# mpriessner/MultiModalSpectralTransformer

Hardware: NVIDIA B200
Metric: generated SMILES tokens/sec (higher is better)
Workload: dtype bf16

## Files before the change

multimodalspectraltransformer_b200/csrc/engine.cu:

```cuda
#include "engine.cuh"
#include "kernels_simt.cuh"
#include "kernels_tc.cuh"
#include "kernels_decode.cuh"
#include "kernels_ffn.cuh"
#include "kernels_attn5.cuh"
#include "kernels_compact.cuh"
#include "kernels_beam.cuh"

#include <algorithm>
#include <cstdlib>
#include <cstring>

namespace mmt {
thread_local std::string g_last_error;

static const char* kEmbedKeys[5] = {
    "linear_spec_embedding_1H.point_embedding_layer_1H.fc_H",
    "linear_spec_embedding_13C.point_embedding_layer_13C.fc_C",
    "linear_spec_embedding_HSQC.point_embedding_layer_HSQC.fc_HSQC",
    "linear_spec_embedding_COSY.point_embedding_layer_COSY.fc_COSY",
    "linear_spec_embedding_IR.linear_spec_embedding_IR"};
static const char* kEncNames[6] = {"encoder_1H", "encoder_13C", "encoder_HSQC", "encoder_COSY", "encoder_IR", "encoder_cross"};

static void prof_pre(mmt_engine* e, cudaStream_t s) {
// ... 129 lines not shown
        void* fn = nullptr;
        cudaDriverEntryPointQueryResult qres;
        MMT_CUDA(cudaGetDriverEntryPoint("cuTensorMapEncodeTiled", &fn, cudaEnableDefault, &qres));
        if (!fn || qres != cudaDriverEntryPointSuccess) MMT_FAIL("cuTensorMapEncodeTiled not available from the driver");
        g_encode_tiled = (PFN_tmapEncodeTiled)fn;
    }
    const int max_smem = TC_MAX_STAGES * TC_STAGE_BYTES_WSPLIT + 1024;
    MMT_CUDA(cudaFuncSetAttribute(gemm_bf16_tc<TC_EPI_STORE>, cudaFuncAttributeMaxDynamicSharedMemorySize, max_smem));
    MMT_CUDA(cudaFuncSetAttribute(gemm_bf16_tc<TC_EPI_LN>, cudaFuncAttributeMaxDynamicSharedMemorySize, max_smem));
    MMT_CUDA(cudaFuncSetAttribute(attn_encoder_tc5, cudaFuncAttributeMaxDynamicSharedMemorySize, A5_SMEM_BYTES));
    MMT_CUDA(cudaFuncSetAttribute(ffn_fused_tc<TC_EPI_STORE, 1>, cudaFuncAttributeMaxDynamicSharedMemorySize, ff_smem_bytes<1>()));
    MMT_CUDA(cudaFuncSetAttribute(ffn_fused_tc<TC_EPI_LN, 1>, cudaFuncAttributeMaxDynamicSharedMemorySize, ff_smem_bytes<1>()));
    MMT_CUDA(cudaFuncSetAttribute(ffn_fused_tc<TC_EPI_STORE, 0>, cudaFuncAttributeMaxDynamicSharedMemorySize, ff_smem_bytes<0>()));
    MMT_CUDA(cudaFuncSetAttribute(ffn_fused_tc<TC_EPI_LN, 0>, cudaFuncAttributeMaxDynamicSharedMemorySize, ff_smem_bytes<0>()));
    MMT_CUDA(cudaFuncSetAttribute(ffn_fused_tc<TC_EPI_LN, 0, 1>, cudaFuncAttributeMaxDynamicSharedMemorySize, ff_smem_bytes<0, 1>()));
    e->tc_ready = true;
    return 0;
}

static int make_tmap(CUtensorMap* m, const __nv_bfloat16* ptr, int64_t rows, int64_t cols, int64_t ld, int box_rows = TC_BM) {
    if (((uintptr_t)ptr & 15) || (ld * 2) % 16) MMT_FAIL("tensor map: operand must be 16-byte aligned with a 16-byte multiple row pitch");
    cuuint64_t dims[2] = {(cuuint64_t)cols, (cuuint64_t)rows};
    cuuint64_t strides[1] = {(cuuint64_t)ld * 2};
    cuuint32_t box[2] = {(cuuint32_t)TC_BK, (cuuint32_t)box_rows};
    cuuint32_t estr[2] = {1, 1};
    CUresult r = g_encode_tiled(m, CU_TENSOR_MAP_DATA_TYPE_BFLOAT16, 2, (void*)ptr, dims, strides, box, estr, CU_TENSOR_MAP_INTERLEAVE_NONE,
                                CU_TENSOR_MAP_SWIZZLE_128B, CU_TENSOR_MAP_L2_PROMOTION_L2_256B, CU_TENSOR_MAP_FLOAT_OOB_FILL_NONE);
    if (r != CUDA_SUCCESS) MMT_FAIL("cuTensorMapEncodeTiled failed with CUresult " + std::to_string((int)r));
    return 0;
}
// ... 73 lines not shown
    }
    if (pro) {
        if (epi != TC_EPI_LN || p.splits != 1 || !pro->W || !pro->out || p.res != pro->out)
            MMT_FAIL("fused FFN prologue needs the LayerNorm epilogue, a weight and the residual buffer as its output");
        p.pro = pro->Wlo ? 2 : 1; p.pro_bias = pro->bias; p.pro_gamma = pro->gamma; p.pro_beta = pro->beta; p.pro_out = pro->out;
        MMT_TRY(make_tmap(&p.tmP, pro->W, D, D, D));
        if (pro->Wlo) MMT_TRY(make_tmap(&p.tmPlo, pro->Wlo, D, D, D));
    }
    dim3 grid(p.splits, (p.M + TC_BM - 1) / TC_BM);
    if (const char* v = getenv("MMT_FFN_KNOCK")) p.knock = atoi(v);
    prof_pre(e, s);
    if (p.wsplit) {
        if (epi == TC_EPI_LN) launch_kernel(ffn_fused_tc<TC_EPI_LN, 1>, grid, dim3(FF_THREADS), ff_smem_bytes<1>(), s, pdl, p);
        else launch_kernel(ffn_fused_tc<TC_EPI_STORE, 1>, grid, dim3(FF_THREADS), ff_smem_bytes<1>(), s, pdl, p);
    } else {
        if (epi == TC_EPI_LN && p.splits == 1 && p.F % (2 * FF_CH) == 0 && e->use_ffn_wide)
            launch_kernel(ffn_fused_tc<TC_EPI_LN, 0, 1>, grid, dim3(ff_threads<0, 1>()), ff_smem_bytes<0, 1>(), s, pdl, p);
        else if (epi == TC_EPI_LN) launch_kernel(ffn_fused_tc<TC_EPI_LN, 0>, grid, dim3(FF_THREADS), ff_smem_bytes<0>(), s, pdl, p);
        else launch_kernel(ffn_fused_tc<TC_EPI_STORE, 0>, grid, dim3(FF_THREADS), ff_smem_bytes<0>(), s, pdl, p);
    }
    return check_launch(e, "ffn_fused_tc", s, 4.0 * p.M * D * p.F);
}

struct ModeLayout {
    int present[5];
    int S_m[5];
    int n_x[5];
    int off[5];
    int S_total;
    int float_mask;
    int has_MF, has_MS, has_MW;
// ... 736 lines not shown

static int decode_self_tail_layer(const DecOps& o, const LayerW& w, bool bf16) {
    const DecBuffers& b = o.b;
    if (bf16) {
        if (o.e->use_gemm_chain && o.Nw <= 24576) {
            const TcChain ch{o.e->Wb(w.ca_in_w), o.plo(w.ca_in_w), w.ca_in_b, b.qc, D};
            MMT_TRY(o.tc_ln(b.att16, D, w.out_w, w.out_b, D, w.n1_w, w.n1_b, &ch));
        } else {
            MMT_TRY(o.tc_ln(b.att16, D, w.out_w, w.out_b, D, w.n1_w, w.n1_b));
            MMT_TRY(o.tc(b.x16, D, w.ca_in_w, w.ca_in_b, b.qc, nullptr, D, D, 0, 1));
        }
    } else {
        MMT_TRY(o.gemm(b.att, D, w.out_w, nullptr, b.part, D, D, 0, 1));
        MMT_TRY(o.ln(b.part, 1, w.out_b, w.n1_w, w.n1_b));
        MMT_TRY(o.gemm(b.x, D, w.ca_in_w, w.ca_in_b, b.qc, D, D, 0, 1));
    }
    return 0;
}

static int decode_cross_tail_layer(const DecOps& o, const LayerW& w, int l, bool bf16, float* x2 = nullptr) {
    mmt_engine* e = o.e;
    const DecBuffers& b = o.b;
    const int M = (int)o.Nw, F = e->desc.d_ff;
    cudaStream_t s = o.s;
    auto keep_x2 = [&]() -> int {
        if (x2) MMT_CUDA(cudaMemcpyAsync(x2, b.x, (size_t)M * D * sizeof(float), cudaMemcpyDeviceToDevice, s));
        return 0;
    };
    if (bf16) {
        const bool ffn_pro = e->use_ffn_prologue && M >= 2048;
// ... 317 lines not shown
        while (early && !stop && checked_polls < n_polls) { MMT_TRY(check_poll(checked_polls)); ++checked_polls; }
        if ((r.mode == 0) && a.stop_on_all_pad && n_waves > 1) {
            for (int i = 0; i < nl; ++i)
                MMT_CUDA(cudaMemcpyAsync(e->h_pinned + i * 128, lb[i].ctl + 8, r.T * sizeof(int), cudaMemcpyDeviceToHost, s));
            MMT_CUDA(cudaStreamSynchronize(s));
            for (int i = 0; i < nl; ++i) for (int q = 0; q < r.T; ++q) nonpad_total[q] += e->h_pinned[i * 128 + q];
        }
    }
    if (staged) {
        MMT_CUDA(cudaMemcpyAsync(r.tokens, st_tokens, (size_t)r.T * N_total * sizeof(int64_t), cudaMemcpyDeviceToDevice, s));
        if (r.probs) MMT_CUDA(cudaMemcpyAsync(r.probs, st_probs, (size_t)r.T * N_total * sizeof(float), cudaMemcpyDeviceToDevice, s));
    }
    if ((r.mode == 0) && a.stop_on_all_pad && n_waves > 1)
        for (int q = 0; q < r.T; ++q) if (nonpad_total[q] == 0) { steps_done = q + 1; break; }
    if (h_steps) *h_steps = steps_done;
    if (e->ffn_dbg) {
        MMT_CUDA(cudaStreamSynchronize(s));
        for (int bshow : {0, 64, 127}) {
            const long long* d = e->ffn_dbg + bshow * 16;
            fprintf(stderr, "ffn_fused_tc<LN> CTA %d: setup %lld | first acc1 %lld | first convert %lld | chunks 8..15:", bshow, d[1] - d[0], d[2] - d[1], d[3] - d[2]);
            for (int i = 9; i <= 15; ++i) fprintf(stderr, " %lld", d[i] - d[i - 1]);
            fprintf(stderr, " | start->acc2 %lld | tmem->stage %lld | LN rows %lld | total %lld\n", d[4] - d[0], d[5] - d[4], d[6] - d[5], d[7] - d[0]);
        }
    }
    if (e->da_dbg) {
        MMT_CUDA(cudaStreamSynchronize(s));
        const int blocks = (int)std::min<int64_t>(4096, (std::min<int64_t>(N_total, max_wave_seqs) + DA_R - 1) / DA_R);
        for (int bshow : {0, blocks / 2, blocks - 1}) {
            fprintf(stderr, "decode_attn phases, CTA %d:", bshow);
            const int last = e->da_dbg[bshow * 16 + 14] ? 14 : 10;
            for (int i = 1; i <= last; ++i) fprintf(stderr, " %lld", e->da_dbg[bshow * 16 + i] - e->da_dbg[bshow * 16 + i - 1]);
            fprintf(stderr, "  total %lld\n", e->da_dbg[bshow * 16 + last] - e->da_dbg[bshow * 16]);
        }
        for (int bshow : {1, blocks / 2}) {
            const long long* d = e->da_dbg + (1024 + bshow) * 16;
            fprintf(stderr, "decode_attn warp 5, CTA %d: self [K+scores %lld | V+acc %lld | reduce %lld | sync %lld]  cross [loop %lld | reduce %lld | sync %lld]\n", bshow,
                    d[1] - d[0], d[2] - d[1], d[3] - d[2], d[4] - d[3], d[6] - d[5], d[7] - d[6], d[8] - d[7]);
        }
        for (int bshow : {0, 33}) {
// ... 172 lines not shown
    if (getenv("MMT_DENSE_ENCODER")) e->use_compact = false;
    if (getenv("MMT_NO_TC_ATTENTION")) e->use_tc_attention = false;
    if (getenv("MMT_TC5_ATTENTION")) e->use_tc5_attention = true;
    if (const char* v = getenv("MMT_FFN_SPLITS")) { int k = atoi(v); if (k == 1 || k == 2 || k == 4 || k == 8 || k == 16 || k == 32) e->ffn_splits_override = k; }
    if (getenv("MMT_TC_ATTENTION_FP32")) e->tc_attention_fp32 = true;
    if (const char* v = getenv("MMT_FUSED_DECODE_ROWS")) e->fused_decode_rows = atoi(v);
    if (getenv("MMT_DEC_FFN_TWO_TERM")) e->dec_ffn_single = false;
    if (getenv("MMT_DEC_PROJ_TWO_TERM")) e->dec_proj_single = false;
    if (const char* v = getenv("MMT_PDL_ROWS")) e->pdl_rows = atoi(v);
    if (getenv("MMT_NO_GEMM_CHAIN")) e->use_gemm_chain = false;
    if (getenv("MMT_NO_FFN_WIDE")) e->use_ffn_wide = false;
    if (getenv("MMT_NO_KV_EPILOGUE")) e->use_kv_epilogue = false;
    if (getenv("MMT_KV_HEAD_MAJOR")) e->kv_tok_major = false;
    if (getenv("MMT_CLUSTER_FFN")) e->use_cluster_ffn = true;
    if (getenv("MMT_NO_FFN_PROLOGUE")) e->use_ffn_prologue = false;
    if (getenv("MMT_ENC_FFN_SINGLE")) e->enc_ffn_single = true;
    if (const char* v = getenv("MMT_DECODE_LANES_LARGE")) e->decode_lanes_large = std::max(1, atoi(v));
    if (const char* v = getenv("MMT_MAX_WAVE_SEQS")) e->max_wave_seqs = std::max(1, atoi(v));
    if (n_floats != e->reg.total) { delete e; MMT_FAIL("weight blob has " + std::to_string(n_floats) + " floats, expected " + std::to_string(build_registry(*desc).total)); }
    auto fail = [&](const std::string& m) { mmt_destroy(e); g_last_error = m; return 1; };
    if (cudaMalloc(&e->w32, n_floats * sizeof(float)) != cudaSuccess) return fail("cudaMalloc weights failed");
    if (cudaMalloc(&e->w16, n_floats * sizeof(__nv_bfloat16)) != cudaSuccess) return fail("cudaMalloc bf16 weights failed");
    if (cudaMemcpy(e->w32, h_weights, n_floats * sizeof(float), cudaMemcpyHostToDevice) != cudaSuccess) return fail("weight H2D copy failed");
    if (cudaMalloc(&e->w16lo, n_floats * sizeof(__nv_bfloat16)) != cudaSuccess) return fail("cudaMalloc bf16 weights (low term) failed");
    f32_to_bf16_split<<<(unsigned)((n_floats + 255) / 256), 256>>>(e->w32, n_floats, e->w16, e->w16lo);
    if (cudaDeviceSynchronize() != cudaSuccess) return fail(std::string("bf16 weight conversion failed: ") + cudaGetErrorString(cudaGetLastError()));
    if (cudaMallocHost(&e->h_pinned, 1024 * sizeof(int32_t)) != cudaSuccess) return fail("cudaMallocHost failed");
    for (int k = 0; k < 6; ++k) {
        e->enc[k].resize(desc->n_enc_layers);
        for (int l = 0; l < desc->n_enc_layers; ++l) fill_layer(e, e->enc[k][l], std::string(kEncNames[k]) + ".layers." + std::to_string(l), false);
// ... 431 lines not shown
            return check_launch(e, "f32_to_bf16", s);
        }
        MMT_CUDA(cudaMemcpyAsync(b.att, src, bytes, cudaMemcpyDeviceToDevice, s));
        return 0;
    };
    const DecOps o{e, b, R, false, s};
    const LayerW& w = e->dec[layer];
    MMT_CUDA(cudaMemcpyAsync(b.x, d_x, bytes, cudaMemcpyDeviceToDevice, s));
    MMT_TRY(load_att(d_att_self));
    MMT_TRY(decode_self_tail_layer(o, w, bf16));
    MMT_CUDA(cudaMemcpyAsync(d_x1, b.x, bytes, cudaMemcpyDeviceToDevice, s));
    MMT_CUDA(cudaMemcpyAsync(d_qc, b.qc, bytes, cudaMemcpyDeviceToDevice, s));
    MMT_TRY(load_att(d_att_cross));
    MMT_TRY(decode_cross_tail_layer(o, w, layer, bf16, d_x2));
    MMT_CUDA(cudaMemcpyAsync(d_out, b.x, bytes, cudaMemcpyDeviceToDevice, s));
    return 0;
}

int32_t mmt_encoder_layer(mmt_engine* e, int32_t stack, int32_t layer, const float* d_x, int64_t rows, int32_t B, int32_t S,
                          const float* d_key_bias, const int32_t* d_row_start, const int32_t* d_cnt, const int32_t* d_kidx,
                          const int32_t* d_nk, int32_t kstride, int32_t precision, float* d_qkv, float* d_att, float* d_out,
                          void* stream) {
    if (!e || !d_x || !d_out) MMT_FAIL("null argument");
    const mmt_model_desc& d = e->desc;
    if (stack < 0 || stack > 5) MMT_FAIL("mmt_encoder_layer: stack must be in [0, 5]");
    if (layer < 0 || layer >= d.n_enc_layers) MMT_FAIL("mmt_encoder_layer: layer out of range");
    if (B <= 0 || B > 65535 || S <= 0 || rows <= 0 || rows > 0x7fffffff) MMT_FAIL("mmt_encoder_layer: empty or oversized batch");
    if (precision != MMT_PREC_FP32 && precision != MMT_PREC_BF16) MMT_FAIL("bad precision");
    const bool ragged = d_key_bias == nullptr;
    if (ragged && (!d_row_start || !d_cnt || !d_kidx || !d_nk || kstride <= 0)) MMT_FAIL("mmt_encoder_layer: the ragged layout needs row_start, cnt, kidx, nk and kstride");
// ... 107 lines not shown
```

multimodalspectraltransformer_b200/csrc/engine.cuh:

```cuda
#pragma once
#include <mutex>
#include <string>
#include <unordered_map>
#include <vector>

#include "../../include/mmt_b200.h"
#include "common.cuh"

namespace mmt {

extern thread_local std::string g_last_error;

#define MMT_FAIL(msg)                                                                   \
    do {                                                                                \
        ::mmt::g_last_error = std::string(__FILE__) + ":" + std::to_string(__LINE__) + ": " + (msg); \
        return 1;                                                                       \
    } while (0)
#define MMT_CUDA(call)                                                                  \
    do {                                                                                \
        cudaError_t err__ = (call);                                                     \
        if (err__ != cudaSuccess) MMT_FAIL(std::string(#call) + " -> " + cudaGetErrorString(err__)); \
    } while (0)
#define MMT_TRY(call)                                                                   \
    do {                                                                                \
// ... 84 lines not shown
    __nv_bfloat16* w16lo = nullptr;
    std::vector<mmt::LayerW> enc[6];
    std::vector<mmt::LayerW> dec;
    char* arena = nullptr;
    size_t arena_bytes = 0;
    int64_t launches = 0;
    bool use_graph = true;
    int fused_decode_rows = 2048;
    int max_wave_seqs = 0;
    bool enc_ffn_single = false;
    bool use_ffn_prologue = true;
    bool use_cluster_ffn = false;
    bool kv_tok_major = true;
    bool use_kv_epilogue = true;
    bool use_ffn_wide = true;
    bool use_gemm_chain = true;
    bool dec_proj_single = true;
    bool sample_ready = false;
    bool dec_ffn_single = true;
    bool use_compact = true;
    struct GraphEntry { std::vector<uint64_t> key; cudaGraphExec_t exec; int64_t launches_per_group; uint64_t stamp; };
    std::vector<GraphEntry> graph_cache;
    uint64_t graph_cache_clock = 0;
    bool use_graph_cache = true;
    bool use_tc_attention = true;
    bool use_tc5_attention = false;
    bool tc_attention_fp32 = false;
    int ffn_splits_override = 0;
    bool use_enc_streams = true;
    cudaStream_t enc_stream[5] = {nullptr, nullptr, nullptr, nullptr, nullptr};
    cudaEvent_t enc_ev[6] = {nullptr, nullptr, nullptr, nullptr, nullptr, nullptr};
    int graph_steps = 16;
    int pdl_rows = 4096;
    bool use_pdl = true;
    cudaStream_t cap_stream[4] = {nullptr, nullptr, nullptr, nullptr};
    cudaEvent_t lane_ev[4] = {nullptr, nullptr, nullptr, nullptr};
    int decode_lanes = 2;
    int decode_lanes_large = 1;
    long long* ffn_dbg = nullptr;
    long long* da_dbg = nullptr;
    bool da_ready = false;
    bool tc_ready = false;
    cudaEvent_t poll_ev[2] = {nullptr, nullptr};
    int32_t* h_pinned = nullptr;
    struct ProfRecord { const char* name; cudaEvent_t a, b; double work; };
    bool profiling = false;
    std::pair<cudaEvent_t, cudaEvent_t> prof_open{nullptr, nullptr};
    std::vector<ProfRecord> prof_records;

    std::mutex mu;
    cudaEvent_t last_use = nullptr;
    cudaStream_t last_stream = nullptr;
    bool last_use_valid = false;

// ... 5 lines not shown
```

multimodalspectraltransformer_b200/csrc/kernels_ffn.cuh:

```cuda
#pragma once
#include "kernels_tc.cuh"

namespace mmt {

constexpr int FF_CH = 64;
constexpr int FF_THREADS = TC_THREADS + 32;
template <int WS, int WIDE> constexpr int ff_threads();
constexpr int FF_X_BYTES = 2 * TC_SLAB_BYTES;
constexpr int FF_H_BYTES = TC_SLAB_BYTES;
constexpr int FF_W1_HALF = FF_CH * 128;
constexpr int FF_W1_STAGE = 2 * TC_SLAB_BYTES;
constexpr int FF_W2_STAGE = 2 * TC_SLAB_BYTES;
constexpr int FF_MAX_F = 2048;
template <int WS, int WIDE> struct FfCfg;
template <> struct FfCfg<1, 0> {
    static constexpr int CH = FF_CH, NB = 2, NS = 2;
    static constexpr int EW = TC_EPI_WARPS;
    static constexpr int W1_STAGE = FF_W1_STAGE, W2_STAGE = FF_W2_STAGE;
    static constexpr int W1_SLAB = TC_SLAB_BYTES;
    static constexpr int W2_KSLAB = 2 * TC_SLAB_BYTES;
    static constexpr int H_BYTES = FF_H_BYTES;
    static constexpr int ACC1_STRIDE = 2 * FF_CH, ACC2_COL = 256;
};
template <> struct FfCfg<0, 0> {
// ... 324 lines not shown
        const float* st = stage_q + (hf * RPW) * TC_LDS;
        if (EPI == TC_EPI_LN) epi_rows_ln(p, st, m0 + q * 32 + hf * RPW, RPW, lane, nullptr, 0, &pre);
        else epi_rows_store(p, st, m0 + q * 32 + hf * RPW, RPW, 0, split, lane);
        if (threadIdx.x == 64) FF_STAMP(6);
    }
    tc_fence_before();
    __syncthreads();
    if (threadIdx.x == 64) FF_STAMP(7);
#undef FF_STAMP
    if (warp == 1) {
        tc_fence_after();
        tmem_dealloc(tmem_base, FF_TMEM_COLS);
    }
}

}
```

multimodalspectraltransformer_b200/csrc/kernels_tc.cuh:

```cuda
#pragma once
#include <cuda.h>

#include "common.cuh"

namespace mmt {

constexpr int TC_BM = 128, TC_BN = 128, TC_BK = 64;
constexpr int TC_SLAB_BYTES = TC_BM * TC_BK * 2;
constexpr int TC_STAGE_BYTES = 2 * TC_SLAB_BYTES;
constexpr int TC_STAGE_BYTES_WSPLIT = 3 * TC_SLAB_BYTES;
constexpr int TC_LDS = TC_BN + 4;
constexpr int TC_STAGING_BYTES = TC_BM * TC_LDS * 4;
constexpr int TC_EPI_WARPS = 8;
constexpr int TC_THREADS = 64 + TC_EPI_WARPS * 32;
constexpr int TC_MAX_STAGES = 4;

enum { TC_EPI_STORE = 0, TC_EPI_LN = 1 };

struct TcGemmParams {
    CUtensorMap tmA;
    CUtensorMap tmW;
    CUtensorMap tmW2;
    int wsplit;
    int M, N, K;
// ... 75 lines not shown
__device__ __forceinline__ void umma_commit(uint64_t* bar) {
    asm volatile("tcgen05.commit.cta_group::1.mbarrier::arrive::one.shared::cluster.b64 [%0];" ::"r"(smem_u32(bar)) : "memory");
}
__device__ __forceinline__ void tmem_ld_32x32(uint32_t taddr, uint32_t (&r)[32]) {
    asm volatile(
        "tcgen05.ld.sync.aligned.32x32b.x32.b32 "
        "{%0, %1, %2, %3, %4, %5, %6, %7, %8, %9, %10, %11, %12, %13, %14, %15, "
        "%16, %17, %18, %19, %20, %21, %22, %23, %24, %25, %26, %27, %28, %29, %30, %31}, [%32];"
        : "=r"(r[0]), "=r"(r[1]), "=r"(r[2]), "=r"(r[3]), "=r"(r[4]), "=r"(r[5]), "=r"(r[6]), "=r"(r[7]),
          "=r"(r[8]), "=r"(r[9]), "=r"(r[10]), "=r"(r[11]), "=r"(r[12]), "=r"(r[13]), "=r"(r[14]), "=r"(r[15]),
          "=r"(r[16]), "=r"(r[17]), "=r"(r[18]), "=r"(r[19]), "=r"(r[20]), "=r"(r[21]), "=r"(r[22]), "=r"(r[23]),
          "=r"(r[24]), "=r"(r[25]), "=r"(r[26]), "=r"(r[27]), "=r"(r[28]), "=r"(r[29]), "=r"(r[30]), "=r"(r[31])
        : "r"(taddr) : "memory");
}
__device__ __forceinline__ void tmem_ld_wait() { asm volatile("tcgen05.wait::ld.sync.aligned;" ::: "memory"); }

__device__ __forceinline__ uint64_t umma_desc_sw128(uint32_t smem_addr) {
    uint64_t d = 0;
    d |= (uint64_t)((smem_addr & 0x3FFFFu) >> 4);
    d |= (uint64_t)1 << 16;
    d |= (uint64_t)(1024 >> 4) << 32;
    d |= (uint64_t)1 << 46;
    d |= (uint64_t)2 << 61;
    return d;
}
__host__ __device__ constexpr uint32_t umma_idesc_bf16(int M, int N) {
    return (1u << 4) | (1u << 7) | (1u << 10) | ((uint32_t)(N >> 3) << 17) | ((uint32_t)(M >> 4) << 24);
}

__device__ __forceinline__ uint2 pack_bf16x4(float4 v) {
    __nv_bfloat162 lo = __floats2bfloat162_rn(v.x, v.y), hi = __floats2bfloat162_rn(v.z, v.w);
    return make_uint2(*reinterpret_cast<uint32_t*>(&lo), *reinterpret_cast<uint32_t*>(&hi));
}

constexpr int EPI_ILP = 8;

template <int NCOLS, int NP = 2>
__device__ __forceinline__ void epi_tmem_to_stage(uint32_t tmem_acc, int q, int hf, int lane, float* stage_q) {
#pragma unroll
    for (int cc = 0; cc < NCOLS / 32 / NP; ++cc) {
        const int c = hf * (NCOLS / 32 / NP) + cc;
        uint32_t r[32];
        tmem_ld_32x32(tmem_acc + ((uint32_t)(q * 32) << 16) + (uint32_t)(c * 32), r);
        tmem_ld_wait();
        float* dst = stage_q + lane * TC_LDS + c * 32;
#pragma unroll
        for (int j = 0; j < 8; ++j)
            *reinterpret_cast<float4*>(dst + 4 * j) =
                make_float4(__uint_as_float(r[4 * j]), __uint_as_float(r[4 * j + 1]), __uint_as_float(r[4 * j + 2]), __uint_as_float(r[4 * j + 3]));
    }
}
template <int EW = TC_EPI_WARPS>
__device__ __forceinline__ void epi_bar_sync() { asm volatile("bar.sync 1, %0;" ::"n"(EW * 32) : "memory"); }

__device__ __forceinline__ void warp_sum_ilp(float (&s)[EPI_ILP]) {
#pragma unroll
    for (int o = 16; o > 0; o >>= 1) {
#pragma unroll
        for (int u = 0; u < EPI_ILP; ++u) s[u] += __shfl_xor_sync(0xffffffffu, s[u], o);
    }
}

struct RowStep {
// ... 15 lines not shown

struct LnPre { float4 bias, ga, be; float4 rs[EPI_ILP]; };
template <class P>
__device__ __forceinline__ void epi_ln_prefetch(const P& p, int row0, int nrows, int lane, LnPre& pre) {
    const int col = lane * 4;
    pre.bias = p.bias ? *reinterpret_cast<const float4*>(p.bias + col) : make_float4(0.f, 0.f, 0.f, 0.f);
    pre.ga = *reinterpret_cast<const float4*>(p.gamma + col);
    pre.be = *reinterpret_cast<const float4*>(p.beta + col);
    const int rows = min(nrows, p.M - row0);
    const float* res = p.res + (int64_t)row0 * D + col;
#pragma unroll
    for (int u = 0; u < EPI_ILP; ++u)
        pre.rs[u] = u < rows ? *reinterpret_cast<const float4*>(res + (int64_t)u * D) : make_float4(0.f, 0.f, 0.f, 0.f);
}

template <class P>
__device__ __forceinline__ void epi_rows_ln(const P& p, const float* stage, int row0, int nrows, int lane, uint8_t* a2 = nullptr, int a2_row0 = 0,
                                            const LnPre* pre = nullptr) {
    const int col = lane * 4;
    float4 bias = make_float4(0.f, 0.f, 0.f, 0.f), ga, be;
    if (pre) { bias = pre->bias; ga = pre->ga; be = pre->be; }
    else {
        if (p.bias) bias = *reinterpret_cast<const float4*>(p.bias + col);
        ga = *reinterpret_cast<const float4*>(p.gamma + col);
        be = *reinterpret_cast<const float4*>(p.beta + col);
    }
    const int rows = min(nrows, p.M - row0);
    if (rows <= 0) return;
    const float* res = p.res + (int64_t)row0 * D + col;
    float* const out32 = p.out_f32 ? p.out_f32 + col : nullptr;
    __nv_bfloat16* const out16 = p.out_b16 ? p.out_b16 + col : nullptr;
    const int64_t ld32 = p.ld_f32, ld16 = p.ld_b16;
    const float eps = p.eps;
    RowStep map(p, row0);
    for (int i0 = 0; i0 < rows; i0 += EPI_ILP) {
        float4 v[EPI_ILP];
        float s[EPI_ILP];
#pragma unroll
        for (int u = 0; u < EPI_ILP; ++u) {
            const bool ok = i0 + u < rows;
            const float4 rs = (pre && i0 == 0) ? pre->rs[u]
                            : ok ? *reinterpret_cast<const float4*>(res + (int64_t)(i0 + u) * D) : make_float4(0.f, 0.f, 0.f, 0.f);
            const float4 a = *reinterpret_cast<const float4*>(stage + (i0 + u) * TC_LDS + col);
            v[u] = make_float4(a.x + bias.x + rs.x, a.y + bias.y + rs.y, a.z + bias.z + rs.z, a.w + bias.w + rs.w);
            s[u] = v[u].x + v[u].y + v[u].z + v[u].w;
        }
        warp_sum_ilp(s);
#pragma unroll
        for (int u = 0; u < EPI_ILP; ++u) {
            const float mean = s[u] * (1.0f / D);
            v[u].x -= mean; v[u].y -= mean; v[u].z -= mean; v[u].w -= mean;
            s[u] = v[u].x * v[u].x + v[u].y * v[u].y + v[u].z * v[u].z + v[u].w * v[u].w;
        }
        warp_sum_ilp(s);
#pragma unroll
        for (int u = 0; u < EPI_ILP; ++u) {
            if (i0 + u < rows) {
                const float rstd = rsqrtf(s[u] * (1.0f / D) + eps);
// ... 247 lines not shown
```

Measured before the change: 17.53 million.

## Add persistent fused FFN kernel overlapping prologue GEMM, FFN and LayerNorm across tiles

Adds a persistent ffn_persist_tc kernel that loops over M tiles with one CTA per SM. Within each CTA it runs the prologue out-projection GEMM plus LN, the two FFN GEMMs, and a final LayerNorm done by dedicated row warps directly from TMEM, all double-buffered so tile k+1's prologue overlaps tile k's tail. The aim is to cut per-CTA setup cost (TMEM alloc, barrier init) and keep tensor cores busy across epilogues. It also adds an XOR-swizzled staging layout to avoid shared-memory bank conflicts, a TMEM store helper and debug stamps. The cost is more complex barrier ring logic, and the dedicated LN warps take three passes over TMEM.

New measurement: 16.99 million, median of 6. 0.969x the previous value.

```diff
diff --git a/multimodalspectraltransformer_b200/csrc/engine.cu b/multimodalspectraltransformer_b200/csrc/engine.cu
--- a/multimodalspectraltransformer_b200/csrc/engine.cu
+++ b/multimodalspectraltransformer_b200/csrc/engine.cu
@@ -167,6 +167,7 @@
     MMT_CUDA(cudaFuncSetAttribute(ffn_fused_tc<TC_EPI_STORE, 0>, cudaFuncAttributeMaxDynamicSharedMemorySize, ff_smem_bytes<0>()));
     MMT_CUDA(cudaFuncSetAttribute(ffn_fused_tc<TC_EPI_LN, 0>, cudaFuncAttributeMaxDynamicSharedMemorySize, ff_smem_bytes<0>()));
     MMT_CUDA(cudaFuncSetAttribute(ffn_fused_tc<TC_EPI_LN, 0, 1>, cudaFuncAttributeMaxDynamicSharedMemorySize, ff_smem_bytes<0, 1>()));
+    MMT_CUDA(cudaFuncSetAttribute(ffn_persist_tc, cudaFuncAttributeMaxDynamicSharedMemorySize, ff_smem_bytes<0, 1>()));
     e->tc_ready = true;
     return 0;
 }
@@ -270,7 +271,17 @@
         if (epi == TC_EPI_LN) launch_kernel(ffn_fused_tc<TC_EPI_LN, 1>, grid, dim3(FF_THREADS), ff_smem_bytes<1>(), s, pdl, p);
         else launch_kernel(ffn_fused_tc<TC_EPI_STORE, 1>, grid, dim3(FF_THREADS), ff_smem_bytes<1>(), s, pdl, p);
     } else {
-        if (epi == TC_EPI_LN && p.splits == 1 && p.F % (2 * FF_CH) == 0 && e->use_ffn_wide)
+        const bool wide = epi == TC_EPI_LN && p.splits == 1 && p.F % (2 * FF_CH) == 0 && e->use_ffn_wide;
+        const bool identity_rows = !p.out_rows && p.S_in == p.M && p.stride_s == 1 && p.off == 0;
+        const bool persist = wide && p.pro == 1 && identity_rows && e->use_ffn_persist;
+        if (p.dbg) {
+            e->ffn_dbg_grid = persist ? (int)std::min<int64_t>(grid.y, e->sm_count) : 0;
+            e->ffn_dbg_tiles = (int)grid.y;
+            if (persist && grid.y > 4096) p.dbg = nullptr;
+        }
+        if (persist) {
+            launch_kernel(ffn_persist_tc, dim3((unsigned)std::min<int64_t>(grid.y, e->sm_count)), dim3(fp_threads()), ff_smem_bytes<0, 1>(), s, pdl, p);
+        } else if (wide)
             launch_kernel(ffn_fused_tc<TC_EPI_LN, 0, 1>, grid, dim3(ff_threads<0, 1>()), ff_smem_bytes<0, 1>(), s, pdl, p);
         else if (epi == TC_EPI_LN) launch_kernel(ffn_fused_tc<TC_EPI_LN, 0>, grid, dim3(FF_THREADS), ff_smem_bytes<0>(), s, pdl, p);
         else launch_kernel(ffn_fused_tc<TC_EPI_STORE, 0>, grid, dim3(FF_THREADS), ff_smem_bytes<0>(), s, pdl, p);
@@ -1037,6 +1048,30 @@
         MMT_TRY(o.gemm(b.att, D, w.out_w, nullptr, b.part, D, D, 0, 1));
         MMT_TRY(o.ln(b.part, 1, w.out_b, w.n1_w, w.n1_b));
         MMT_TRY(o.gemm(b.x, D, w.ca_in_w, w.ca_in_b, b.qc, D, D, 0, 1));
+    }
+    return 0;
+}
+
+static int print_ffn_stamps(mmt_engine* e, cudaStream_t s) {
+    MMT_CUDA(cudaStreamSynchronize(s));
+    if (e->ffn_dbg_grid == 0) {
+        for (int bshow : {0, 64, 127}) {
+            const long long* d = e->ffn_dbg + bshow * 16;
+            fprintf(stderr, "ffn_fused_tc<LN> CTA %d: setup %lld | first acc1 %lld | first convert %lld | chunks 8..15:", bshow, d[1] - d[0], d[2] - d[1], d[3] - d[2]);
+            for (int i = 9; i <= 15; ++i) fprintf(stderr, " %lld", d[i] - d[i - 1]);
+            fprintf(stderr, " | start->acc2 %lld | tmem->stage %lld | LN rows %lld | total %lld\n", d[4] - d[0], d[5] - d[4], d[6] - d[5], d[7] - d[0]);
+        }
+        return 0;
+    }
+    const int G = e->ffn_dbg_grid;
+    const long long t0 = e->ffn_dbg[0];
+    for (int t = 0; t < e->ffn_dbg_tiles; t += G) {
+        const long long* d = e->ffn_dbg + (int64_t)t * FP_DBG_SLOTS;
+        fprintf(stderr, "ffn_persist_tc CTA 0 tile %d: prologue GEMM %lld | LN2 %lld..%lld | first acc1 %lld | chunk cadence:", t, d[0] - t0, d[1] - t0, d[2] - t0, d[3] - t0);
+        for (int i = 5; i <= 11; ++i) fprintf(stderr, " %lld", d[i] - d[i - 1]);
+        fprintf(stderr, " | last conversion %lld | LN3 %lld..%lld", d[11] - t0, d[12] - t0, d[13] - t0);
+        if (t + G < e->ffn_dbg_tiles) fprintf(stderr, " | tile period %lld", e->ffn_dbg[(int64_t)(t + G) * FP_DBG_SLOTS + 1] - d[1]);
+        fprintf(stderr, "\n");
     }
     return 0;
 }
@@ -1384,15 +1419,7 @@
     if ((r.mode == 0) && a.stop_on_all_pad && n_waves > 1)
         for (int q = 0; q < r.T; ++q) if (nonpad_total[q] == 0) { steps_done = q + 1; break; }
     if (h_steps) *h_steps = steps_done;
-    if (e->ffn_dbg) {
-        MMT_CUDA(cudaStreamSynchronize(s));
-        for (int bshow : {0, 64, 127}) {
-            const long long* d = e->ffn_dbg + bshow * 16;
-            fprintf(stderr, "ffn_fused_tc<LN> CTA %d: setup %lld | first acc1 %lld | first convert %lld | chunks 8..15:", bshow, d[1] - d[0], d[2] - d[1], d[3] - d[2]);
-            for (int i = 9; i <= 15; ++i) fprintf(stderr, " %lld", d[i] - d[i - 1]);
-            fprintf(stderr, " | start->acc2 %lld | tmem->stage %lld | LN rows %lld | total %lld\n", d[4] - d[0], d[5] - d[4], d[6] - d[5], d[7] - d[0]);
-        }
-    }
+    if (e->ffn_dbg) MMT_TRY(print_ffn_stamps(e, s));
     if (e->da_dbg) {
         MMT_CUDA(cudaStreamSynchronize(s));
         const int blocks = (int)std::min<int64_t>(4096, (std::min<int64_t>(N_total, max_wave_seqs) + DA_R - 1) / DA_R);
@@ -1595,6 +1622,7 @@
     if (getenv("MMT_KV_HEAD_MAJOR")) e->kv_tok_major = false;
     if (getenv("MMT_CLUSTER_FFN")) e->use_cluster_ffn = true;
     if (getenv("MMT_NO_FFN_PROLOGUE")) e->use_ffn_prologue = false;
+    if (getenv("MMT_NO_FFN_PERSIST")) e->use_ffn_persist = false;
     if (getenv("MMT_ENC_FFN_SINGLE")) e->enc_ffn_single = true;
     if (const char* v = getenv("MMT_DECODE_LANES_LARGE")) e->decode_lanes_large = std::max(1, atoi(v));
     if (const char* v = getenv("MMT_MAX_WAVE_SEQS")) e->max_wave_seqs = std::max(1, atoi(v));
@@ -2056,6 +2084,7 @@
     MMT_TRY(load_att(d_att_cross));
     MMT_TRY(decode_cross_tail_layer(o, w, layer, bf16, d_x2));
     MMT_CUDA(cudaMemcpyAsync(d_out, b.x, bytes, cudaMemcpyDeviceToDevice, s));
+    if (e->ffn_dbg && layer == 3) MMT_TRY(print_ffn_stamps(e, s));
     return 0;
 }
 
diff --git a/multimodalspectraltransformer_b200/csrc/engine.cuh b/multimodalspectraltransformer_b200/csrc/engine.cuh
--- a/multimodalspectraltransformer_b200/csrc/engine.cuh
+++ b/multimodalspectraltransformer_b200/csrc/engine.cuh
@@ -122,6 +122,7 @@
     bool kv_tok_major = true;
     bool use_kv_epilogue = true;
     bool use_ffn_wide = true;
+    bool use_ffn_persist = true;
     bool use_gemm_chain = true;
     bool dec_proj_single = true;
     bool sample_ready = false;
@@ -146,6 +147,7 @@
     int decode_lanes = 2;
     int decode_lanes_large = 1;
     long long* ffn_dbg = nullptr;
+    int ffn_dbg_grid = 0, ffn_dbg_tiles = 0;
     long long* da_dbg = nullptr;
     bool da_ready = false;
     bool tc_ready = false;
diff --git a/multimodalspectraltransformer_b200/csrc/kernels_ffn.cuh b/multimodalspectraltransformer_b200/csrc/kernels_ffn.cuh
--- a/multimodalspectraltransformer_b200/csrc/kernels_ffn.cuh
+++ b/multimodalspectraltransformer_b200/csrc/kernels_ffn.cuh
@@ -362,4 +362,331 @@
     }
 }
 
+constexpr int FP_ROW_WARPS = 4;
+constexpr int fp_threads() { return ff_threads<0, 1>() + 32 * FP_ROW_WARPS; }
+constexpr int FP_DBG_SLOTS = 16;
+
+__device__ __forceinline__ void ln_row_thread(const FfnParams& p, uint32_t tacc, int grow) {
+    const bool ok = grow < p.M;
+    const float* res = p.res + (int64_t)(ok ? grow : 0) * D;
+    auto tree = [](float (&s)[16]) {
+#pragma unroll
+        for (int o = 8; o > 0; o >>= 1)
+#pragma unroll
+            for (int L = 0; L < o; ++L) s[L] += s[L + o];
+        return s[0];
+    };
+    float s[16];
+#pragma unroll
+    for (int cg = 0; cg < 4; ++cg) {
+        uint32_t a[32];
+        tmem_ld_32x32(tacc + (uint32_t)(cg * 32), a);
+        tmem_ld_wait();
+#pragma unroll
+        for (int j = 0; j < 8; ++j) {
+            const int col = cg * 32 + 4 * j;
+            const float4 bias = p.bias ? *reinterpret_cast<const float4*>(p.bias + col) : make_float4(0.f, 0.f, 0.f, 0.f);
+            const float4 rs = ok ? *reinterpret_cast<const float4*>(res + col) : make_float4(0.f, 0.f, 0.f, 0.f);
+            const float4 x = make_float4(__uint_as_float(a[4 * j]), __uint_as_float(a[4 * j + 1]), __uint_as_float(a[4 * j + 2]), __uint_as_float(a[4 * j + 3]));
+            const float4 v = make_float4(x.x + bias.x + rs.x, x.y + bias.y + rs.y, x.z + bias.z + rs.z, x.w + bias.w + rs.w);
+            const float t = v.x + v.y + v.z + v.w;
+            if (cg < 2) s[cg * 8 + j] = t; else s[(cg - 2) * 8 + j] += t;
+            a[4 * j] = __float_as_uint(v.x); a[4 * j + 1] = __float_as_uint(v.y); a[4 * j + 2] = __float_as_uint(v.z); a[4 * j + 3] = __float_as_uint(v.w);
+        }
+        tmem_st_32x32(tacc + (uint32_t)(cg * 32), a);
+    }
+    tmem_st_wait();
+    const float mean = tree(s) * (1.0f / D);
+#pragma unroll
+    for (int cg = 0; cg < 4; ++cg) {
+        uint32_t a[32];
+        tmem_ld_32x32(tacc + (uint32_t)(cg * 32), a);
+        tmem_ld_wait();
+#pragma unroll
+        for (int j = 0; j < 8; ++j) {
+            float4 v = make_float4(__uint_as_float(a[4 * j]), __uint_as_float(a[4 * j + 1]), __uint_as_float(a[4 * j + 2]), __uint_as_float(a[4 * j + 3]));
+            v.x -= mean; v.y -= mean; v.z -= mean; v.w -= mean;
+            const float t = v.x * v.x + v.y * v.y + v.z * v.z + v.w * v.w;
+            if (cg < 2) s[cg * 8 + j] = t; else s[(cg - 2) * 8 + j] += t;
+        }
+    }
+    const float rstd = rsqrtf(tree(s) * (1.0f / D) + p.eps);
+#pragma unroll
+    for (int cg = 0; cg < 4; ++cg) {
+        uint32_t a[32];
+        tmem_ld_32x32(tacc + (uint32_t)(cg * 32), a);
+        tmem_ld_wait();
+#pragma unroll
+        for (int j = 0; j < 8; ++j) {
+            float4 v = make_float4(__uint_as_float(a[4 * j]), __uint_as_float(a[4 * j + 1]), __uint_as_float(a[4 * j + 2]), __uint_as_float(a[4 * j + 3]));
+            v.x -= mean; v.y -= mean; v.z -= mean; v.w -= mean;
+            const int col = cg * 32 + 4 * j;
+            const float4 ga = *reinterpret_cast<const float4*>(p.gamma + col), be = *reinterpret_cast<const float4*>(p.beta + col);
+            const float4 o = make_float4(v.x * rstd * ga.x + be.x, v.y * rstd * ga.y + be.y, v.z * rstd * ga.z + be.z, v.w * rstd * ga.w + be.w);
+            if (ok) {
+                if (p.out_f32) *reinterpret_cast<float4*>(p.out_f32 + (int64_t)grow * p.ld_f32 + col) = o;
+                if (p.out_b16) *reinterpret_cast<uint2*>(p.out_b16 + (int64_t)grow * p.ld_b16 + col) = pack_bf16x4(o);
+            }
+        }
+    }
 }
+
+__global__ void __launch_bounds__(fp_threads(), 1) ffn_persist_tc(const __grid_constant__ FfnParams p) {
+    typedef FfCfg<0, 1> C;
+    constexpr int NB = C::NB, NS = C::NS, CH = C::CH;
+    constexpr int EW = C::EW, NP = EW / 4, RPW = 32 / NP;
+    constexpr int G2_WARP = 2 + EW, ROW_WARP0 = G2_WARP + 1;
+    constexpr int R = 12;
+    static_assert(R % NS == 0 && R % NB == 0, "barrier ring must be a multiple of both buffer counts");
+    static_assert(NB * C::H_BYTES == TC_BM * TC_BN * 4, "the LN2 staging tile fills the H buffers exactly");
+    static_assert(2 * C::ACC1_STRIDE + 2 * TC_BN == FF_TMEM_COLS, "TMEM: acc1 2 x 128 | acc2 2 x 128");
+    extern __shared__ uint8_t smem_raw[];
+    __shared__ __align__(8) uint64_t x_full, w1_full[NS], w2_full[NS], h_full[NB], acc1_free[NB], g1_done[R], g2_done[R];
+    __shared__ __align__(8) uint64_t pro_acc_full[2], x2_ready[2], acc2_full[2], acc2_free[2];
+    __shared__ uint32_t tmem_slot;
+
+    uint8_t* smem = smem_raw + ((1024u - (smem_u32(smem_raw) & 1023u)) & 1023u);
+    uint8_t* sX = smem;
+    uint8_t* sH = sX + FF_X_BYTES;
+    uint8_t* sW = sH + NB * C::H_BYTES;
+    uint8_t* sW2 = sW + NS * C::W1_STAGE;
+    const int warp = threadIdx.x >> 5, lane = threadIdx.x & 31;
+    const int n = p.F / CH;
+    const int tiles = (p.M + TC_BM - 1) / TC_BM;
+    const int my_tiles = (tiles - (int)blockIdx.x + (int)gridDim.x - 1) / (int)gridDim.x;
+    auto tile_of = [&](int k) { return (int)blockIdx.x + k * (int)gridDim.x; };
+#define FP_STAMP(k, i) do { if (p.dbg) p.dbg[tile_of(k) * FP_DBG_SLOTS + (i)] = clock64(); } while (0)
+    pdl_launch_dependents();
+
+    if (warp == 0 && lane == 0) {
+        tma_prefetch_desc(&p.tmX); tma_prefetch_desc(&p.tmW1); tma_prefetch_desc(&p.tmW2); tma_prefetch_desc(&p.tmP);
+        mbar_init(&x_full, 1);
+        for (int s = 0; s < NS; ++s) { mbar_init(&w1_full[s], 1); mbar_init(&w2_full[s], 1); }
+        for (int s = 0; s < NB; ++s) { mbar_init(&acc1_free[s], EW); mbar_init(&h_full[s], EW); }
+        for (int s = 0; s < R; ++s) { mbar_init(&g1_done[s], 1); mbar_init(&g2_done[s], 1); }
+        for (int b = 0; b < 2; ++b) { mbar_init(&pro_acc_full[b], 1); mbar_init(&x2_ready[b], EW); mbar_init(&acc2_full[b], 1); mbar_init(&acc2_free[b], FP_ROW_WARPS); }
+        fence_barrier_init();
+    }
+    if (warp == 1) tmem_alloc(&tmem_slot, FF_TMEM_COLS);
+    tc_fence_before();
+    __syncthreads();
+    tc_fence_after();
+    const uint32_t tmem_base = tmem_slot;
+    auto acc2_of = [&](int k) { return tmem_base + C::ACC2_COL + (uint32_t)((k & 1) * TC_BN); };
+    auto w1_item_done = [&](int g) {
+        const int k = g / (n + 1), j = g - k * (n + 1);
+        if (j == 0) mbar_wait(&pro_acc_full[k & 1], ((uint32_t)(k >> 1)) & 1u);
+        else { const int i = k * n + j - 1; mbar_wait(&g1_done[i % R], ((uint32_t)(i / R)) & 1u); }
+    };
+
+    if (warp == 0) {
+        if (lane == 0) {
+            int g = 0;
+            for (int k = 0; k < my_tiles; ++k) {
+                const int m0 = tile_of(k) * TC_BM, i0 = k * n;
+                {
+                    const int s = g % NS;
+                    if (g >= NS) w1_item_done(g - NS);
+                    mbar_arrive_expect_tx(&w1_full[s], 2 * TC_SLAB_BYTES);
+                    for (int ks = 0; ks < 2; ++ks) tma_load_2d(sW + (size_t)s * C::W1_STAGE + ks * C::W1_SLAB, &p.tmP, &w1_full[s], ks * TC_BK, 0);
+                    ++g;
+                }
+                if (k == 0) pdl_wait();
+                else mbar_wait(&g1_done[(i0 - 1) % R], ((uint32_t)((i0 - 1) / R)) & 1u);
+                mbar_arrive_expect_tx(&x_full, FF_X_BYTES);
+                tma_load_2d(sX, &p.tmX, &x_full, 0, m0);
+                tma_load_2d(sX + TC_SLAB_BYTES, &p.tmX, &x_full, TC_BK, m0);
+                for (int it = 0; it <= n; ++it) {
+                    if (it < n) {
+                        const int s = g % NS, c = it;
+                        if (g >= NS) w1_item_done(g - NS);
+                        mbar_arrive_expect_tx(&w1_full[s], C::W1_STAGE);
+                        uint8_t* w = sW + (size_t)s * C::W1_STAGE;
+#pragma unroll
+                        for (int rh = 0; rh < CH / FF_CH; ++rh) {
+                            tma_load_2d(w + rh * FF_W1_HALF, &p.tmW1, &w1_full[s], 0, c * CH + rh * FF_CH);
+                            tma_load_2d(w + C::W1_SLAB + rh * FF_W1_HALF, &p.tmW1, &w1_full[s], TC_BK, c * CH + rh * FF_CH);
+                        }
+                        ++g;
+                    }
+                    if (it >= 1) {
+                        const int c = it - 1, i = i0 + c, s = i % NS;
+                        if (i >= NS) mbar_wait(&g2_done[(i - NS) % R], ((uint32_t)((i - NS) / R)) & 1u);
+                        mbar_arrive_expect_tx(&w2_full[s], C::W2_STAGE);
+                        uint8_t* w = sW2 + (size_t)s * C::W2_STAGE;
+#pragma unroll
+                        for (int ks = 0; ks < CH / FF_CH; ++ks) tma_load_2d(w + ks * C::W2_KSLAB, &p.tmW2, &w2_full[s], c * CH + ks * FF_CH, 0);
+                    }
+                }
+            }
+        }
+    } else if (warp == 1) {
+        if (lane == 0) {
+            const uint32_t idesc1 = umma_idesc_bf16(TC_BM, CH), idescP = umma_idesc_bf16(TC_BM, TC_BN);
+            const uint32_t x_addr = smem_u32(sX);
+            int g = 0;
+            for (int k = 0; k < my_tiles; ++k) {
+                const int b2 = k & 1;
+                {
+                    const int s = g % NS;
+                    mbar_wait(&w1_full[s], ((uint32_t)(g / NS)) & 1u);
+                    mbar_wait(&x_full, (uint32_t)k & 1u);
+                    if (k >= 2) mbar_wait(&acc2_free[b2], ((uint32_t)((k - 2) >> 1)) & 1u);
+                    tc_fence_after();
+                    if (threadIdx.x == 32) FP_STAMP(k, 0);
+                    const uint32_t wp = smem_u32(sW + (size_t)s * C::W1_STAGE);
+                    for (int ks = 0; ks < 2; ++ks) {
+                        const uint64_t adesc = umma_desc_sw128(x_addr + ks * TC_SLAB_BYTES);
+                        const uint64_t bdesc = umma_desc_sw128(wp + ks * C::W1_SLAB);
+#pragma unroll
+                        for (int kk = 0; kk < TC_BK / 16; ++kk)
+                            umma_bf16(acc2_of(k), adesc + (uint64_t)(2 * kk), bdesc + (uint64_t)(2 * kk), idescP, (ks > 0 || kk > 0) ? 1u : 0u);
+                    }
+                    umma_commit(&pro_acc_full[b2]);
+                    ++g;
+                }
+                mbar_wait(&x2_ready[b2], ((uint32_t)(k >> 1)) & 1u);
+                tc_fence_after();
+                for (int c = 0; c < n; ++c) {
+                    const int i = k * n + c, s = g % NS;
+                    mbar_wait(&w1_full[s], ((uint32_t)(g / NS)) & 1u);
+                    if (i >= NB) mbar_wait(&acc1_free[i % NB], ((uint32_t)((i - NB) / NB)) & 1u);
+                    tc_fence_after();
+                    const uint32_t w1 = smem_u32(sW + (size_t)s * C::W1_STAGE);
+                    const uint32_t acc1 = tmem_base + (uint32_t)((i % NB) * C::ACC1_STRIDE);
+#pragma unroll
+                    for (int kk = 0; kk < D / 16; ++kk) {
+                        const uint64_t adesc = umma_desc_sw128(x_addr + (kk >> 2) * TC_SLAB_BYTES) + (uint64_t)(2 * (kk & 3));
+                        const uint64_t bdesc = umma_desc_sw128(w1 + (kk >> 2) * C::W1_SLAB) + (uint64_t)(2 * (kk & 3));
+                        umma_bf16(acc1, adesc, bdesc, idesc1, kk > 0 ? 1u : 0u);
+                    }
+                    umma_commit(&g1_done[i % R]);
+                    ++g;
+                }
+            }
+        }
+    } else if (warp == G2_WARP) {
+        if (lane == 0) {
+            const uint32_t idesc2 = umma_idesc_bf16(TC_BM, TC_BN);
+            for (int k = 0; k < my_tiles; ++k) {
+                for (int c = 0; c < n; ++c) {
+                    const int j = k * n + c, b = j % NB, sw = j % NS;
+                    mbar_wait(&w2_full[sw], ((uint32_t)(j / NS)) & 1u);
+                    mbar_wait(&h_full[b], ((uint32_t)(j / NB)) & 1u);
+                    tc_fence_after();
+                    const uint32_t h_addr = smem_u32(sH + (size_t)b * C::H_BYTES), w2_addr = smem_u32(sW2 + (size_t)sw * C::W2_STAGE);
+#pragma unroll
+                    for (int kk = 0; kk < CH / 16; ++kk) {
+                        const uint64_t adesc = umma_desc_sw128(h_addr + (kk >> 2) * TC_SLAB_BYTES) + (uint64_t)(2 * (kk & 3));
+                        const uint64_t bdesc = umma_desc_sw128(w2_addr + (kk >> 2) * C::W2_KSLAB) + (uint64_t)(2 * (kk & 3));
+                        umma_bf16(acc2_of(k), adesc, bdesc, idesc2, (c > 0 || kk > 0) ? 1u : 0u);
+                    }
+                    umma_commit(&g2_done[j % R]);
+                }
+                umma_commit(&acc2_full[k & 1]);
+            }
+        }
+    } else if (warp < G2_WARP) {
+        const int q = warp & 3, hf = (warp - 2) >> 2;
+        const int row = q * 32 + lane;
+        constexpr int CPW = CH / NP;
+        for (int k = 0; k < my_tiles; ++k) {
+            const int m0 = tile_of(k) * TC_BM, i0 = k * n, b2 = k & 1;
+            {
+                LnView v{p.pro_bias, p.pro_gamma, p.pro_beta, p.res, p.pro_out, nullptr, D, D, p.M, p.eps, nullptr, p.M > 0 ? p.M : 1, 0, 1, 0};
+                if (k == 0) pdl_wait();
+                LnPre pre;
+                epi_ln_prefetch(v, m0 + q * 32 + hf * RPW, RPW, lane, pre);
+                mbar_wait(&pro_acc_full[b2], ((uint32_t)(k >> 1)) & 1u);
+                if (k > 0) mbar_wait(&g2_done[(i0 - 1) % R], ((uint32_t)((i0 - 1) / R)) & 1u);
+                tc_fence_after();
+                if (threadIdx.x == 64) FP_STAMP(k, 1);
+                float* stage = reinterpret_cast<float*>(sH);
+                epi_tmem_to_stage<TC_BN, NP, true>(acc2_of(k), q, hf, lane, stage + (q * 32) * TC_BN);
+                epi_bar_sync<EW>();
+                epi_rows_ln<LnView, true>(v, stage + (q * 32 + hf * RPW) * TC_BN, m0 + q * 32 + hf * RPW, RPW, lane, sX, q * 32 + hf * RPW, &pre);
+                fence_proxy_async_smem();
+                tc_fence_before();
+                __syncwarp();
+                if (lane == 0) mbar_arrive(&x2_ready[b2]);
+                if (threadIdx.x == 64) FP_STAMP(k, 2);
+            }
+            for (int c = 0; c < n; ++c) {
+                const int i = i0 + c, b = i % NB;
+                float4 bias[CPW / 32][8];
+#pragma unroll
+                for (int cc = 0; cc < CPW / 32; ++cc) {
+                    const float4* bsrc = reinterpret_cast<const float4*>(p.b1 + (size_t)c * CH + hf * CPW + cc * 32);
+#pragma unroll
+                    for (int j = 0; j < 8; ++j) bias[cc][j] = __ldg(bsrc + j);
+                }
+                mbar_wait(&g1_done[i % R], ((uint32_t)(i / R)) & 1u);
+                tc_fence_after();
+                if (threadIdx.x == 64 && c == 0) FP_STAMP(k, 3);
+                uint32_t pk[CPW / 2];
+                {
+                    uint32_t r[CPW / 32][32];
+#pragma unroll
+                    for (int cc = 0; cc < CPW / 32; ++cc)
+                        tmem_ld_32x32(tmem_base + ((uint32_t)(q * 32) << 16) + (uint32_t)(b * C::ACC1_STRIDE + hf * CPW + cc * 32), r[cc]);
+                    tmem_ld_wait();
+                    tc_fence_before();
+                    __syncwarp();
+                    if (lane == 0) mbar_arrive(&acc1_free[b]);
+#pragma unroll
+                    for (int cc = 0; cc < CPW / 32; ++cc) {
+                        const float4* bb = bias[cc];
+#pragma unroll
+                        for (int j = 0; j < 8; ++j) {
+                            float v0 = __uint_as_float(r[cc][4 * j]), v1 = __uint_as_float(r[cc][4 * j + 1]), v2 = __uint_as_float(r[cc][4 * j + 2]), v3 = __uint_as_float(r[cc][4 * j + 3]);
+                            v0 = fmaxf(v0 + bb[j].x, 0.f); v1 = fmaxf(v1 + bb[j].y, 0.f); v2 = fmaxf(v2 + bb[j].z, 0.f); v3 = fmaxf(v3 + bb[j].w, 0.f);
+                            __nv_bfloat162 lo = __floats2bfloat162_rn(v0, v1), hi = __floats2bfloat162_rn(v2, v3);
+                            pk[cc * 16 + 2 * j] = *reinterpret_cast<uint32_t*>(&lo);
+                            pk[cc * 16 + 2 * j + 1] = *reinterpret_cast<uint32_t*>(&hi);
+                        }
+                    }
+                }
+                if (i >= NB) mbar_wait(&g2_done[(i - NB) % R], ((uint32_t)((i - NB) / R)) & 1u);
+#pragma unroll
+                for (int cc = 0; cc < CPW / 32; ++cc) {
+                    const int col0 = hf * CPW + cc * 32;
+                    uint8_t* hrow = sH + (size_t)b * C::H_BYTES + (size_t)(col0 >> 6) * TC_SLAB_BYTES + (size_t)row * 128;
+#pragma unroll
+                    for (int c4 = 0; c4 < 4; ++c4) {
+                        const int cj = ((col0 & 63) >> 3) + c4;
+                        *reinterpret_cast<uint4*>(hrow + ((cj ^ (row & 7)) << 4)) = make_uint4(pk[cc * 16 + 4 * c4], pk[cc * 16 + 4 * c4 + 1], pk[cc * 16 + 4 * c4 + 2], pk[cc * 16 + 4 * c4 + 3]);
+                    }
+                }
+                fence_proxy_async_smem();
+                tc_fence_before();
+                __syncwarp();
+                if (lane == 0) mbar_arrive(&h_full[b]);
+                if (threadIdx.x == 64 && c >= n - 8) FP_STAMP(k, 12 - n + c);
+            }
+        }
+    } else {
+        const int q = warp & 3;
+        pdl_wait();
+        for (int k = 0; k < my_tiles; ++k) {
+            const int b2 = k & 1;
+            mbar_wait(&x2_ready[b2], ((uint32_t)(k >> 1)) & 1u);
+            mbar_wait(&acc2_full[b2], ((uint32_t)(k >> 1)) & 1u);
+            tc_fence_after();
+            if (warp == ROW_WARP0 && lane == 0) FP_STAMP(k, 12);
+            ln_row_thread(p, acc2_of(k) + ((uint32_t)(q * 32) << 16), tile_of(k) * TC_BM + q * 32 + lane);
+            tc_fence_before();
+            __syncwarp();
+            if (lane == 0) mbar_arrive(&acc2_free[b2]);
+            if (warp == ROW_WARP0 && lane == 0) FP_STAMP(k, 13);
+        }
+    }
+    tc_fence_before();
+    __syncthreads();
+#undef FP_STAMP
+    if (warp == 1) {
+        tc_fence_after();
+        tmem_dealloc(tmem_base, FF_TMEM_COLS);
+    }
+}
+
+}
diff --git a/multimodalspectraltransformer_b200/csrc/kernels_tc.cuh b/multimodalspectraltransformer_b200/csrc/kernels_tc.cuh
--- a/multimodalspectraltransformer_b200/csrc/kernels_tc.cuh
+++ b/multimodalspectraltransformer_b200/csrc/kernels_tc.cuh
@@ -113,6 +113,17 @@
         : "r"(taddr) : "memory");
 }
 __device__ __forceinline__ void tmem_ld_wait() { asm volatile("tcgen05.wait::ld.sync.aligned;" ::: "memory"); }
+__device__ __forceinline__ void tmem_st_32x32(uint32_t taddr, const uint32_t (&r)[32]) {
+    asm volatile(
+        "tcgen05.st.sync.aligned.32x32b.x32.b32 [%0], "
+        "{%1, %2, %3, %4, %5, %6, %7, %8, %9, %10, %11, %12, %13, %14, %15, %16, "
+        "%17, %18, %19, %20, %21, %22, %23, %24, %25, %26, %27, %28, %29, %30, %31, %32};"
+        :: "r"(taddr), "r"(r[0]), "r"(r[1]), "r"(r[2]), "r"(r[3]), "r"(r[4]), "r"(r[5]), "r"(r[6]), "r"(r[7]),
+          "r"(r[8]), "r"(r[9]), "r"(r[10]), "r"(r[11]), "r"(r[12]), "r"(r[13]), "r"(r[14]), "r"(r[15]),
+          "r"(r[16]), "r"(r[17]), "r"(r[18]), "r"(r[19]), "r"(r[20]), "r"(r[21]), "r"(r[22]), "r"(r[23]),
+          "r"(r[24]), "r"(r[25]), "r"(r[26]), "r"(r[27]), "r"(r[28]), "r"(r[29]), "r"(r[30]), "r"(r[31]) : "memory");
+}
+__device__ __forceinline__ void tmem_st_wait() { asm volatile("tcgen05.wait::st.sync.aligned;" ::: "memory"); }
 
 __device__ __forceinline__ uint64_t umma_desc_sw128(uint32_t smem_addr) {
     uint64_t d = 0;
@@ -134,7 +145,7 @@
 
 constexpr int EPI_ILP = 8;
 
-template <int NCOLS, int NP = 2>
+template <int NCOLS, int NP = 2, bool SWZ = false>
 __device__ __forceinline__ void epi_tmem_to_stage(uint32_t tmem_acc, int q, int hf, int lane, float* stage_q) {
 #pragma unroll
     for (int cc = 0; cc < NCOLS / 32 / NP; ++cc) {
@@ -142,10 +153,10 @@
         uint32_t r[32];
         tmem_ld_32x32(tmem_acc + ((uint32_t)(q * 32) << 16) + (uint32_t)(c * 32), r);
         tmem_ld_wait();
-        float* dst = stage_q + lane * TC_LDS + c * 32;
+        float* dst = SWZ ? stage_q + lane * TC_BN : stage_q + lane * TC_LDS + c * 32;
 #pragma unroll
         for (int j = 0; j < 8; ++j)
-            *reinterpret_cast<float4*>(dst + 4 * j) =
+            *reinterpret_cast<float4*>(dst + (SWZ ? ((c * 8 + j) ^ lane) * 4 : 4 * j)) =
                 make_float4(__uint_as_float(r[4 * j]), __uint_as_float(r[4 * j + 1]), __uint_as_float(r[4 * j + 2]), __uint_as_float(r[4 * j + 3]));
     }
 }
@@ -191,7 +202,7 @@
         pre.rs[u] = u < rows ? *reinterpret_cast<const float4*>(res + (int64_t)u * D) : make_float4(0.f, 0.f, 0.f, 0.f);
 }
 
-template <class P>
+template <class P, bool SWZ = false>
 __device__ __forceinline__ void epi_rows_ln(const P& p, const float* stage, int row0, int nrows, int lane, uint8_t* a2 = nullptr, int a2_row0 = 0,
                                             const LnPre* pre = nullptr) {
     const int col = lane * 4;
@@ -218,7 +229,8 @@
             const bool ok = i0 + u < rows;
             const float4 rs = (pre && i0 == 0) ? pre->rs[u]
                             : ok ? *reinterpret_cast<const float4*>(res + (int64_t)(i0 + u) * D) : make_float4(0.f, 0.f, 0.f, 0.f);
-            const float4 a = *reinterpret_cast<const float4*>(stage + (i0 + u) * TC_LDS + col);
+            const float4 a = SWZ ? *reinterpret_cast<const float4*>(stage + (i0 + u) * TC_BN + ((lane ^ ((a2_row0 + i0 + u) & 31)) << 2))
+                                 : *reinterpret_cast<const float4*>(stage + (i0 + u) * TC_LDS + col);
             v[u] = make_float4(a.x + bias.x + rs.x, a.y + bias.y + rs.y, a.z + bias.z + rs.z, a.w + bias.w + rs.w);
             s[u] = v[u].x + v[u].y + v[u].z + v[u].w;
         }
```
